# Wuziyi616/LEOD

Hardware: AMD Instinct MI355X
Metric: event-frames/sec/GPU (RVT-S train, Gen1 T=21) at 1/2/4/8 GPUs; mAP@0.5 parity (higher is better)
Workload: dtype fp16

## Files before the change

leod_amd/csrc/k_linear_wgrad.hip:

```cpp
#include "linear_common.hpp"
#include "wgrad_bf16.hpp"
#include "wgrad_dma.hpp"

LEOD_API long leod_workspace_bytes() { return (long)kWgwScratchBytes; }
LEOD_API int leod_set_workspace(void* ws, long bytes, hipStream_t stream) {
    if (ws && (bytes <= 0 || (reinterpret_cast<uintptr_t>(ws) & 15))) return LEOD_ERR_ARG;
    wgrad_wide_register_scratch(stream, ws, (size_t)(bytes > 0 ? bytes : 0));
    return LEOD_OK;
}

__global__ void leod_family_marker_kernel(int begin) { (void)begin; }
struct FamilyMarker {
    hipStream_t s; bool on;
    explicit FamilyMarker(hipStream_t st) : s(st) {
        static const bool env = getenv("LEOD_FAMILY_MARKERS") && atoi(getenv("LEOD_FAMILY_MARKERS"));
        on = env;
        if (on) hipLaunchKernelGGL(leod_family_marker_kernel, dim3(1), dim3(1), 0, s, 1);
    }
    ~FamilyMarker() { if (on) hipLaunchKernelGGL(leod_family_marker_kernel, dim3(1), dim3(1), 0, s, 0); }
};

static int route_linear_wgrad(const float* dy, long lddy, int dyfmt, const XRows& xl, float* dW, float* dbias, int M, int N, int K,
                              hipStream_t stream) {
    const int xm = xl.x_mode();
    if (xm == XM_BF16 || xm == XM_F16) {
        if (xl.stats || xl.x2) return LEOD_ERR_ARG;
        if (!use_wgrad_wide(xl, lddy, M, N, K, dyfmt) && !wgrad_dma_ok(xl, lddy, M, N, K, dyfmt)) return LEOD_ERR_UNSUPPORTED;
    }
    if (wgrad_dma_ok(xl, lddy, M, N, K, dyfmt)) {
        const int rc = launch_wgrad_dma(dy, lddy, xl, dW, (long)K, dbias, M, N, K, stream, dyfmt);
        if (rc != LEOD_ERR_UNSUPPORTED) return rc;
// ... 63 lines not shown
```

leod_amd/csrc/wgrad_bf16.hpp:

```cpp
#pragma once

typedef unsigned u4_ __attribute__((ext_vector_type(4)));

__device__ __forceinline__ f2_ gelu_erf2(f2_ x) {
    const f2_ z = __builtin_elementwise_abs(x) * 0.70710678118654752440f;
    const f2_ d = z * 0.3275911f + 1.0f;
    const f2_ t = {fast_rcp(d.x), fast_rcp(d.y)};
    const f2_ poly = t * (0.254829592f + t * (-0.284496736f + t * (1.421413741f + t * (-1.453152027f + t * 1.061405429f))));
    const f2_ a = (z * z) * -1.4426950408889634f;
    const f2_ e = {__builtin_amdgcn_exp2f(a.x), __builtin_amdgcn_exp2f(a.y)};
    const f2_ ht = (0.5f * poly) * e;
    const f2_ cdf = {x.x >= 0.f ? 1.0f - ht.x : ht.x, x.y >= 0.f ? 1.0f - ht.y : ht.y};
    return x * cdf;
}
__device__ __forceinline__ unsigned pack_bf16x2(f2_ v) { return __builtin_bit_cast(unsigned, __builtin_convertvector(v, bf2_)); }

constexpr int wgw_row_groups(int slots_per_row) {
    int g = 1;
    while (2 * g * slots_per_row <= 256) g *= 2;
    return g;
}
template <int RG, int T, int BST>
__device__ __forceinline__ constexpr int wgw_slot_off(int e) {
    return RG >= 16 ? e * (RG / 16) * T * BST : (e % (16 / (RG < 16 ? RG : 16))) * RG * 16 + (e / (16 / (RG < 16 ? RG : 16))) * T * BST;
}

template <int TN, int TK, int RC, int MS = 1>
constexpr int wgw_lds_bytes() {
    return 2 * ((RC / 16) * (TN + TK) * 272) * 2 > (MS - 1) * 12 * 1024 ? 2 * ((RC / 16) * (TN + TK) * 272) * 2 : (MS - 1) * 12 * 1024;
}

template <int TN, int TK, int NWN, int NWK, int RC, int DYF, int XM, int OCC>
__global__ __launch_bounds__(256, OCC) void wgrad_wide_bf16_kernel(const void* __restrict__ dyv, long lddy, XRows xl, float* dW, long ldw,
                                                                    float* dbias, f4* __restrict__ part, int M, int N, int K, int dbg) {
    constexpr int WA = TN / NWN, WB = TK / NWK, MS = 4 / (NWN * NWK), KS = RC / 32;
    constexpr bool K16 = KS % MS != 0;
    constexpr int NSL = WA * WB + WA;
    static_assert((WA == 3 || WA == 6) && (WB == 3 || WB == 6) && WA * WB <= 18 && NWN * NWK * MS == 4 && (RC / 16) % MS == 0 &&
                  (MS == 1 || (WA == 3 && WB == 3)), "4 waves of 3 x 3, 6 x 3 or 3 x 6 tiles");
    constexpr int BST = 16 * 16 + 16;
    constexpr int DCW = DYF ? 8 : 4, XCW = XM >= XM_GELU16 ? 8 : 4;
    constexpr int DSPR = 16 * TN / DCW, XSPR = 16 * TK / XCW;
    constexpr int DRG = wgw_row_groups(DSPR) < RC ? wgw_row_groups(DSPR) : RC, XRG = wgw_row_groups(XSPR) < RC ? wgw_row_groups(XSPR) : RC;
    constexpr bool XG = XM == XM_GELU16;
    static_assert(!XG || (RC * XSPR) % 256 == 0, "whole slots per thread");
    constexpr int RN = RC / DRG, RK = XG ? RC * XSPR / 256 : RC / XRG;
    constexpr int SDY = (RC / 16) * TN * BST, SX = (RC / 16) * TK * BST;
    static_assert(DSPR * DRG == 192 && (XG || XSPR * XRG == 192), "three waves stage an operand");
    static_assert(2 * (SDY + SX) * 2 <= wgw_lds_bytes<TN, TK, RC, MS>(), "LDS size");
    extern __shared__ __attribute__((aligned(16))) unsigned short wg_smem[];
    const int tid = threadIdx.x, lane = tid & 63, wave = __builtin_amdgcn_readfirstlane(tid >> 6);
    const int i = lane & 15, q = lane >> 4;
    const int wn = wave % NWN, wk = (wave / NWN) % NWK, ws = wave / (NWN * NWK);
    const int n0 = blockIdx.y * TN * 16, k0 = blockIdx.z * TK * 16;
    const bool dact = wave < 3, xact = XG || wave >= 1;
    const int xt = tid - 64;
    const int dcs = tid % DSPR, drg = tid / DSPR, xcs = (xact ? xt : 0) % XSPR, xrg = (xact ? xt : 0) / XSPR;
// ... 186 lines not shown
    }
    __syncthreads();
    int buf = 0;
    for (; m0 < M; m0 += mstride) {
        const long mn = m0 + mstride;
        const bool more = mn < M;
        if (more) { if (mn + RC <= M) fetch(mn, FULL); else fetch(mn, TAILC); }
        if (!(dbg & 2)) mfma_chunk(buf);
        if (more) stash(mn, buf ^ 1);
        __syncthreads();
        buf ^= 1;
    }
    if constexpr (MS > 1) {
        f4* sred = reinterpret_cast<f4*>(wg_smem);
        if (ws > 0) {
#pragma unroll
            for (int a = 0; a < WA; ++a) {
#pragma unroll
                for (int b = 0; b < WB; ++b) sred[((ws - 1) * NSL + a * WB + b) * 64 + lane] = acc[a][b];
                sred[((ws - 1) * NSL + WA * WB + a) * 64 + lane] = bacc[a];
            }
        }
        __syncthreads();
        if (ws > 0) return;
#pragma unroll
        for (int o = 0; o < MS - 1; ++o)
#pragma unroll
            for (int a = 0; a < WA; ++a) {
#pragma unroll
                for (int b = 0; b < WB; ++b) acc[a][b] += sred[(o * NSL + a * WB + b) * 64 + lane];
                bacc[a] += sred[(o * NSL + WA * WB + a) * 64 + lane];
            }
    }
    if (dbg & 1) return;
    if constexpr (XM == XM_LN) {
#pragma unroll
        for (int b = 0; b < WB; ++b) {
            const int k = k0 + 16 * (wk * WB + b) + i;
            const float g = k < K ? xl.ln_w[k] : 0.f, sh = k < K ? xl.ln_b[k] : 0.f;
#pragma unroll
            for (int a = 0; a < WA; ++a)
#pragma unroll
                for (int r = 0; r < 4; ++r) acc[a][b][r] = fmaf(g, acc[a][b][r], sh * bacc[a][r]);
        }
    }
    const bool bias_out = dbias != nullptr && blockIdx.z == 0;
    if (part != nullptr) {
        constexpr int NW = NWN * NWK;
        const long tile = (long)blockIdx.y * gridDim.z + blockIdx.z, ntiles = (long)gridDim.y * gridDim.z;
        f4* dst = part + (((long)blockIdx.x * ntiles + tile) * NW + (wk * NWN + wn)) * (NSL * 64) + lane;
#pragma unroll
        for (int a = 0; a < WA; ++a) {
#pragma unroll
            for (int b = 0; b < WB; ++b) dst[(a * WB + b) * 64] = acc[a][b];
            if (bias_out && a % NWK == wk) dst[(WA * WB + a) * 64] = bacc[a];
        }
        return;
    }
#pragma unroll
    for (int b = 0; b < WB; ++b) {
        const int k = k0 + 16 * (wk * WB + b) + i;
#pragma unroll
        for (int a = 0; a < WA; ++a)
#pragma unroll
            for (int r = 0; r < 4; ++r) {
                const int n = n0 + 16 * (wn * WA + a) + 4 * q + r;
                if (n < N && k < K) atomicAdd(dW + (long)n * ldw + k, acc[a][b][r]);
            }
    }
    if (bias_out && i == 0) {
#pragma unroll
        for (int a = 0; a < WA; ++a)
            if (a % NWK == wk) {
#pragma unroll
                for (int r = 0; r < 4; ++r) {
                    const int n = n0 + 16 * (wn * WA + a) + 4 * q + r;
                    if (n < N) atomicAdd(dbias + n, bacc[a][r]);
                }
            }
    }
}

template <int TN, int TK, int NWN, int NWK>
__global__ __launch_bounds__(256) void wgrad_wide_reduce_kernel(const f4* __restrict__ part, int gx, int ny, int nz, int per, float* dW, long ldw,
                                                                float* dbias, int N, int K) {
    constexpr int NW = NWN * NWK, WA = TN / NWN, WB = TK / NWK, NT9 = WA * WB, NSL = NT9 + WA;
    const long O = (long)ny * nz * NW * NSL * 64;
    const long o = (long)blockIdx.x * 256 + threadIdx.x;
    if (o >= O) return;
    const int lane = (int)(o & 63), t = (int)((o >> 6) % NSL), w = (int)((o / (64 * NSL)) % NW), tile = (int)(o / (64 * NSL * NW));
    const int ty = tile / nz, tz = tile - ty * nz, wn = w % NWN, wk = w / NWN, i = lane & 15, q = lane >> 4;
    if (t >= NT9 && !(dbias != nullptr && tz == 0 && (t - NT9) % NWK == wk && i == 0)) return;
    const int g0 = blockIdx.y * per, g1 = min(gx, g0 + per);
    f4 s0 = zero4(), s1 = zero4(), s2 = zero4(), s3 = zero4();
    const f4* p = part + (long)g0 * O + o;
    int g = g0;
    f4 s4 = zero4(), s5 = zero4(), s6 = zero4(), s7 = zero4();
    for (; g + 8 <= g1; g += 8, p += 8 * O) {
        s0 += p[0]; s1 += p[O]; s2 += p[2 * O]; s3 += p[3 * O]; s4 += p[4 * O]; s5 += p[5 * O]; s6 += p[6 * O]; s7 += p[7 * O];
    }
    for (; g + 4 <= g1; g += 4, p += 4 * O) { s0 += p[0]; s1 += p[O]; s2 += p[2 * O]; s3 += p[3 * O]; }
    for (; g < g1; ++g, p += O) s0 += p[0];
    const f4 v = ((s0 + s1) + (s2 + s3)) + ((s4 + s5) + (s6 + s7));
    const bool single = gridDim.y == 1;
    if (t < NT9) {
        const int a = t / WB, b = t - a * WB;
        const int k = tz * TK * 16 + 16 * (wk * WB + b) + i;
#pragma unroll
        for (int r = 0; r < 4; ++r) {
            const int n = ty * TN * 16 + 16 * (wn * WA + a) + 4 * q + r;
            if (n < N && k < K) {
                float* d = dW + (long)n * ldw + k;
                if (single) *d += v[r]; else atomicAdd(d, v[r]);
            }
        }
    } else {
#pragma unroll
        for (int r = 0; r < 4; ++r) {
            const int n = ty * TN * 16 + 16 * (wn * WA + (t - NT9)) + 4 * q + r;
            if (n < N) { if (single) dbias[n] += v[r]; else atomicAdd(dbias + n, v[r]); }
        }
    }
}

#include <mutex>
#include <unordered_map>
struct WgwScratch { void* p = nullptr; size_t bytes = 0; };
static inline std::unordered_map<hipStream_t, WgwScratch>& wgw_scratch_map() { static std::unordered_map<hipStream_t, WgwScratch> m; return m; }
static inline std::mutex& wgw_scratch_mutex() { static std::mutex m; return m; }
constexpr size_t kWgwScratchBytes = (size_t)768 << 20;
static inline void wgrad_wide_register_scratch(hipStream_t s, void* p, size_t bytes) {
    std::lock_guard<std::mutex> lock(wgw_scratch_mutex());
    WgwScratch& e = wgw_scratch_map()[s];
    e.p = p; e.bytes = p ? bytes : 0;
}
static inline f4* wgrad_wide_scratch(hipStream_t s, size_t bytes) {
    std::lock_guard<std::mutex> lock(wgw_scratch_mutex());
    WgwScratch& e = wgw_scratch_map()[s];
    if (e.bytes >= bytes) return reinterpret_cast<f4*>(e.p);
    hipStreamCaptureStatus cs = hipStreamCaptureStatusNone;
    if (hipStreamIsCapturing(s, &cs) != hipSuccess || cs != hipStreamCaptureStatusNone) { (void)hipGetLastError(); return nullptr; }
    void* nb = nullptr;
    const size_t want = bytes < kWgwScratchBytes ? kWgwScratchBytes : bytes;
    if (hipMalloc(&nb, want) != hipSuccess) { (void)hipGetLastError(); return nullptr; }
    e.p = nb; e.bytes = want;
    return reinterpret_cast<f4*>(nb);
}

template <int TN, int TK, int NWN, int NWK, int RC, int DYF, int XM, int OCC>
static inline int launch_wgrad_wide_cfg(const void* dy, long lddy, const XRows& xl, float* dW, long ldw, float* dbias,
                                        int M, int N, int K, hipStream_t s) {
    constexpr int dbg = 0;
    constexpr int LDS = wgw_lds_bytes<TN, TK, RC, 4 / (NWN * NWK)>();
    const int tiles = cdiv(N, TN * 16) * cdiv(K, TK * 16), chunks = cdiv(M, RC);
    const int wgs = M <= 60000 ? 384 : OCC * 256;
    int gx = max(1, min(chunks / 2, wgs / tiles));
    if (gx >= 16) gx &= ~7;
    dim3 grid(gx, cdiv(N, TN * 16), cdiv(K, TK * 16));
    auto kern = wgrad_wide_bf16_kernel<TN, TK, NWN, NWK, RC, DYF, XM, OCC>;
    static bool attr_set = false;
    if (!attr_set) { hipFuncSetAttribute(reinterpret_cast<const void*>(kern), hipFuncAttributeMaxDynamicSharedMemorySize, LDS); attr_set = true; }
    constexpr int NW = NWN * NWK, NSL = (TN / NWN) * (TK / NWK) + TN / NWN;
    const long O = (long)tiles * NW * NSL * 64;
    f4* part = gx > 1 ? wgrad_wide_scratch(s, (size_t)gx * O * sizeof(f4)) : nullptr;
    hipLaunchKernelGGL(kern, grid, dim3(256), LDS, s, dy, lddy, xl, dW, ldw, dbias, part, M, N, K, dbg);
    if (part != nullptr && !(dbg & 1)) {
        const int ob = (int)cdiv(O, 256);
        int groups = max(1, min(gx, 512 / ob));
        const int per = cdiv(gx, groups);
        groups = cdiv(gx, per);
        hipLaunchKernelGGL((wgrad_wide_reduce_kernel<TN, TK, NWN, NWK>), dim3(ob, groups), dim3(256), 0, s, part, gx, (int)grid.y, (int)grid.z, per,
                           dW, ldw, dbias, N, K);
    }
    return leod_launch_status();
}

static inline int wgrad_wide_combo(const XRows& xl, int N, int K, int dyfmt) {
    const int xm = xl.x_mode();
    if (xm == XM_F16) {
        if (dyfmt) return 0;
        if (N <= 48 && K <= 48) return 14;
        if (K <= 48 || N <= 48) return 0;
        return (K % 192 == 0 && N >= 96) ? 16 : 15;
    }
    const bool f32_rows = !dyfmt && xm == XM_ROWS, f32_gelu = !dyfmt && xm == XM_GELU16, f32_bf16 = !dyfmt && xm == XM_BF16;
    const bool b16_rows = dyfmt && xm == XM_ROWS, b16_ln = dyfmt && xm == XM_LN;
    if (N <= 48 && K <= 48) return f32_rows ? 1 : f32_bf16 ? 8 : 0;
    if (K <= 48) return b16_ln ? 2 : 0;
    if (N <= 48) return f32_gelu ? 3 : 0;
    if (N % 192 == 0 && K >= 96 && (b16_ln || b16_rows)) return b16_ln ? 10 : 11;
    if (K % 192 == 0 && N >= 96 && (f32_gelu || f32_bf16)) return f32_gelu ? 12 : 13;
    return f32_rows ? 4 : b16_ln ? 5 : f32_gelu ? 6 : b16_rows ? 7 : f32_bf16 ? 9 : 0;
}
static inline bool use_wgrad_wide(const XRows& xl, long lddy, int M, int N, int K, int dyfmt) {
    if (leod_precision() != 1 || M < 8192) return false;
    const int xm = xl.x_mode();
// ... 31 lines not shown
```

leod_amd/csrc/wgrad_dma.hpp:

```cpp
#pragma once

struct Prep16 {
    const void* src; long ld;
    const float* src2; long ld2; int C1;
    const float* stats;
    unsigned short* dst;
    int C, mode;
};
enum Prep16Mode : int { P16_NONE = -1, P16_F32 = 0, P16_LN = 1 , P16_GELU16 = 2, P16_F16 = 3, P16_CONCAT = 4  };
static inline int prep16_mode(int xm, bool concat) {
    if (xm_is_mfma_operand(xm)) return P16_NONE;
    return xm == XM_LN ? P16_LN : xm == XM_GELU16 ? P16_GELU16 : xm == XM_F16 ? P16_F16 : concat ? P16_CONCAT : P16_F32;
}

struct Prep16Group { Prep16 a[4]; Prep16 b[4]; };
__global__ __launch_bounds__(256) void wgrad_prep16_kernel(Prep16Group grp, int M) {
    const Prep16& p = blockIdx.y ? grp.b[blockIdx.z] : grp.a[blockIdx.z];
    if (p.mode < 0) return;
    const int C8 = p.C >> 3;
    const long it = (long)blockIdx.x * 256 + threadIdx.x;
    if (it >= (long)M * C8) return;
    const long m = it / C8;
    const int c = (int)(it - m * C8) << 3;
    f4 lo, hi;
// ... 6 lines not shown
    } else {
        const float* s = (p.mode == 4 && c >= p.C1) ? p.src2 + m * p.ld2 + (c - p.C1) : reinterpret_cast<const float*>(p.src) + m * p.ld + c;
        lo = ld4(s); hi = ld4(s + 4);
        if (p.mode == 1) {
            const f2_ st = *reinterpret_cast<const f2_*>(p.stats + 2 * m);
            lo = (lo - st.x) * st.y; hi = (hi - st.x) * st.y;
        }
    }
    const u4_ o = {pack_bf16x2(f2_{lo.x, lo.y}), pack_bf16x2(f2_{lo.z, lo.w}), pack_bf16x2(f2_{hi.x, hi.y}), pack_bf16x2(f2_{hi.z, hi.w})};
    *reinterpret_cast<u4_*>(p.dst + m * p.C + c) = o;
}

__device__ __forceinline__ void wgd_dma16(const void* gsrc, unsigned lds_dst) {
    unsigned keep;
    asm volatile("s_mov_b32 %0, m0\n\ts_mov_b32 m0, %2\n\ts_nop 0\n\tglobal_load_lds_dwordx4 %1, off\n\ts_mov_b32 m0, %0"
                 : "=&s"(keep) : "v"(gsrc), "s"(lds_dst) : "memory");
}
template <int N> __device__ __forceinline__ void wgd_wait_vm() { asm volatile("s_waitcnt vmcnt(%0)" :: "n"(N) : "memory"); }

template <int T, int RC, int NS> constexpr int wgd_lds_bytes() { return NS * 2 * (RC / 16) * T * 256 * 2; }
template <int T, int RC, int NS> constexpr int wgd_occupancy() { return wgd_lds_bytes<T, RC, NS>() <= 52 * 1024 ? 3 : wgd_lds_bytes<T, RC, NS>() <= 80 * 1024 ? 2 : 1; }

struct WgdProb {
    const unsigned short* A; long lda; const unsigned short* B; long ldb; const float* ln_w; const float* ln_b; float* dbias_flag; f4* part;
    int cpw, gx, ny, nz, N, K, blk0;
};
struct WgdGroup { WgdProb p[4]; int n; };
template <int T, int RC, int NS, bool LN>
__global__ __launch_bounds__(256, ((wgd_occupancy<T, RC, NS>()) >= 2 ? 2 : 1)) void wgrad_dma_kernel(WgdGroup grp, int chunks, int dbg) {
    int pk = 0;
    for (int k = 1; k < grp.n; ++k) if ((int)blockIdx.x >= grp.p[k].blk0) pk = k;
    const WgdProb& pr = grp.p[pk];
    const unsigned short* __restrict__ A = pr.A; const unsigned short* __restrict__ B = pr.B; const long lda = pr.lda, ldb = pr.ldb;
    const float* __restrict__ ln_w = pr.ln_w; const float* __restrict__ ln_b = pr.ln_b; float* dbias_flag = pr.dbias_flag; f4* __restrict__ part = pr.part;
    const int cpw = pr.cpw, gx = pr.gx, ny = pr.ny, nz = pr.nz, K = pr.K;
    const int bid = (int)blockIdx.x - pr.blk0;
    const bool ln = LN && ln_w != nullptr;
    constexpr int WA = T / 2, WB = T / 2, NWN = 2, NWK = 2, RB = RC / 16, KS = RC / 32;
    constexpr int BLK = 256;
    constexpr int SA = RB * T * BLK, SLOT = 2 * SA;
    constexpr int NI = SLOT * 2 / 1024, IPW = NI / 4;
    static_assert(NI % 4 == 0 && RC % 32 == 0, "whole instructions per wave");
    constexpr int NSL = WA * WB + WA;
    extern __shared__ __attribute__((aligned(1024))) unsigned short wd_smem[];
    const int tid = threadIdx.x, lane = tid & 63, wave = __builtin_amdgcn_readfirstlane(tid >> 6);
    const int i = lane & 15, q = lane >> 4;
    const int wn = wave % NWN, wk = wave / NWN;
    const int ntl = ny * nz;
    int tl, bx;
    if ((gx & 7) == 0) { const int xcd = bid & 7, sj = bid >> 3; tl = sj % ntl; bx = (sj / ntl) * 8 + xcd; }
    else { bx = bid % gx; tl = bid / gx; }
    const int by = tl / nz, bz = tl - by * nz;
    const int n0 = by * T * 16, k0 = bz * T * 16;
    const int c0 = bx * cpw, c1 = min(chunks, c0 + cpw);
    const int nch = c1 - c0;
    static_assert(IPW % 2 == 0, "the first half of a wave's instructions fills the dY part, the second half the X part");
    const char* src[IPW];
    const long stepA = (long)RC * lda * 2, stepB = (long)RC * ldb * 2;
#pragma unroll
    for (int j = 0; j < IPW; ++j) {
        const int t = wave + 4 * j;
        const int blk = 2 * t + (lane >> 5), r = (lane & 31) >> 1, half = lane & 1;
        const bool isb = j >= IPW / 2;
        const int b = isb ? blk - RB * T : blk;
        const int rb = b / T, cb = b - rb * T;
        const long ld = isb ? ldb : lda;
        const int col = (isb ? k0 : n0) + cb * 16 + half * 8;
        src[j] = reinterpret_cast<const char*>(isb ? B : A) + (((long)c0 * RC + rb * 16 + r) * ld + col) * 2;
    }
    const unsigned lds0 = __builtin_amdgcn_readfirstlane((unsigned)(size_t)wd_smem);
    auto issue = [&](int slot) {
#pragma unroll
        for (int j = 0; j < IPW; ++j) {
            wgd_dma16(src[j], __builtin_amdgcn_readfirstlane(lds0 + (unsigned)(slot * SLOT * 2 + (wave + 4 * j) * 1024)));
            src[j] += j >= IPW / 2 ? stepB : stepA;
        }
    };
    const bool bias_out = dbias_flag != nullptr && bz == 0;
    const bool bias_any = ln || bias_out;
    f4 acc[WA][WB], bacc[WA];
#pragma unroll
    for (int a = 0; a < WA; ++a) {
        bacc[a] = zero4();
#pragma unroll
        for (int b = 0; b < WB; ++b) acc[a][b] = zero4();
    }
    const s8v ones = {0x3F80, 0x3F80, 0x3F80, 0x3F80, 0x3F80, 0x3F80, 0x3F80, 0x3F80};
    typedef __attribute__((address_space(3))) s4 lds_s4;
    const int loff = (4 * q + (i >> 2)) * 16 + 4 * (i & 3);
    auto mfma_chunk = [&](int slot) {
        const unsigned short* pdy = wd_smem + slot * SLOT + (wn * WA) * BLK + loff;
        const unsigned short* px = wd_smem + slot * SLOT + SA + (wk * WB) * BLK + loff;
#pragma unroll
        for (int ks = 0; ks < KS; ++ks) {
            const int st = 2 * ks;
            s8v pa[WA], pb[WB];
#pragma unroll
            for (int a = 0; a < WA; ++a) {
                const s4 lo = __builtin_amdgcn_ds_read_tr16_b64_v4i16((lds_s4*)(pdy + (st * T + a) * BLK));
                const s4 hi = __builtin_amdgcn_ds_read_tr16_b64_v4i16((lds_s4*)(pdy + ((st + 1) * T + a) * BLK));
                pa[a] = __builtin_shufflevector(lo, hi, 0, 1, 2, 3, 4, 5, 6, 7);
// ... 25 lines not shown
        if (c + NS - 1 < nch && !(dbg & 2)) issue((c + NS - 1) % NS);
        if (!(dbg & 1)) mfma_chunk(c % NS);
    }
    if (ln) {
#pragma unroll
        for (int b = 0; b < WB; ++b) {
            const int k = k0 + 16 * (wk * WB + b) + i;
            const float g = k < K ? ln_w[k] : 0.f, sh = k < K ? ln_b[k] : 0.f;
#pragma unroll
            for (int a = 0; a < WA; ++a)
#pragma unroll
                for (int r = 0; r < 4; ++r) acc[a][b][r] = fmaf(g, acc[a][b][r], sh * bacc[a][r]);
        }
    }
    constexpr int NW = NWN * NWK;
    const long tile = (long)by * nz + bz, ntiles = ntl;
    f4* dst = part + (((long)bx * ntiles + tile) * NW + (wk * NWN + wn)) * (NSL * 64) + lane;
#pragma unroll
    for (int a = 0; a < WA; ++a) {
#pragma unroll
        for (int b = 0; b < WB; ++b) dst[(a * WB + b) * 64] = acc[a][b];
        if (bias_out && a % NWK == wk) dst[(WA * WB + a) * 64] = bacc[a];
    }
}

constexpr int kWgdRC = 64;
constexpr size_t kWgdOperandBytes = (size_t)600 << 20;

static inline int wgd_tile(int N, int K) {
    if (N % 96 == 0 && K % 96 == 0) return 6;
    if (N % 128 == 0 && K % 128 == 0) return 8;
    if (N % 64 == 0 && K % 64 == 0) return 4;
    return 0;
}
static inline bool wgrad_dma_ok(const XRows& xl, long lddy, int M, int N, int K, int dyfmt) {
    if (leod_precision() != 1 || M < 8192 || (M % kWgdRC) || N < 64 || K < 64) return false;
    const int T = wgd_tile(N, K);
    if (!T) return false;
    const int xm = xl.x_mode();
    if ((lddy & 7) || (xl.ld & 7)) return false;
    if (xl.x2 && (xm != XM_ROWS || (xl.K1 & 7) || (xl.ld2 & 7))) return false;
    const size_t need = (size_t)M * ((dyfmt ? 0 : N) + (xm_is_mfma_operand(xm) ? 0 : K)) * 2;
    if (need > kWgdOperandBytes) return false;
    if (M > (T == 6 ? 60000 : 400000)) return false;
    if (!dyfmt && xm != XM_BF16 && xm != XM_GELU16 && (long)N * K < 200000) return false;
    return true;
}

struct WgrProb { const f4* part; float* dW; float* dbias; long ldw; int gx, ny, nz, per, N, K, ob, groups; };
struct WgrGroup { WgrProb p[4]; };
template <int T>
__global__ __launch_bounds__(256) void wgrad_dma_reduce_kernel(WgrGroup grp) {
    const WgrProb& pr = grp.p[blockIdx.z];
    if ((int)blockIdx.x >= pr.ob || (int)blockIdx.y >= pr.groups) return;
    constexpr int NWN = 2, NWK = 2, NW = 4, WA = T / 2, WB = T / 2, NT9 = WA * WB, NSL = NT9 + WA;
    const int gx = pr.gx, nz = pr.nz, per = pr.per, N = pr.N, K = pr.K;
    float* dW = pr.dW; float* dbias = pr.dbias; const long ldw = pr.ldw;
    const long O = (long)pr.ny * nz * NW * NSL * 64;
    const long o = (long)blockIdx.x * 256 + threadIdx.x;
    if (o >= O) return;
    const int lane = (int)(o & 63), t = (int)((o >> 6) % NSL), w = (int)((o / (64 * NSL)) % NW), tile = (int)(o / (64 * NSL * NW));
    const int ty = tile / nz, tz = tile - ty * nz, wn = w % NWN, wk = w / NWN, i = lane & 15, q = lane >> 4;
    if (t >= NT9 && !(dbias != nullptr && tz == 0 && (t - NT9) % NWK == wk && i == 0)) return;
    const int g0 = blockIdx.y * per, g1 = min(gx, g0 + per);
    f4 s0 = zero4(), s1 = zero4(), s2 = zero4(), s3 = zero4(), s4 = zero4(), s5 = zero4(), s6 = zero4(), s7 = zero4();
    const f4* p = pr.part + (long)g0 * O + o;
    int g = g0;
    for (; g + 8 <= g1; g += 8, p += 8 * O) {
        s0 += p[0]; s1 += p[O]; s2 += p[2 * O]; s3 += p[3 * O]; s4 += p[4 * O]; s5 += p[5 * O]; s6 += p[6 * O]; s7 += p[7 * O];
    }
    for (; g + 4 <= g1; g += 4, p += 4 * O) { s0 += p[0]; s1 += p[O]; s2 += p[2 * O]; s3 += p[3 * O]; }
    for (; g < g1; ++g, p += O) s0 += p[0];
    const f4 v = ((s0 + s1) + (s2 + s3)) + ((s4 + s5) + (s6 + s7));
    const bool single = pr.groups == 1;
    if (t < NT9) {
        const int a = t / WB, b = t - a * WB;
        const int k = tz * T * 16 + 16 * (wk * WB + b) + i;
#pragma unroll
        for (int r = 0; r < 4; ++r) {
            const int n = ty * T * 16 + 16 * (wn * WA + a) + 4 * q + r;
            if (n < N && k < K) {
                float* d = dW + (long)n * ldw + k;
                if (single) *d += v[r]; else atomicAdd(d, v[r]);
            }
        }
    } else {
#pragma unroll
        for (int r = 0; r < 4; ++r) {
            const int n = ty * T * 16 + 16 * (wn * WA + (t - NT9)) + 4 * q + r;
            if (n < N) { if (single) dbias[n] += v[r]; else atomicAdd(dbias + n, v[r]); }
        }
    }
}

struct WgdHostProb { const void* dy; long lddy; XRows xl; float* dW; long ldw; float* dbias; int N, K, dyfmt; };

template <int T, int RC, int NS>
static inline int launch_wgrad_dma_group_t(int n, const WgdHostProb* hp, int M, hipStream_t s) {
    constexpr int TW = T * 16;
    constexpr int LDS = wgd_lds_bytes<T, RC, NS>();
    constexpr int dbg = 0;
    constexpr int NW = 4, NSL = (T / 2) * (T / 2) + T / 2;
    const int chunks = M / RC;
    const int target = 256 * wgd_occupancy<T, RC, NS>();
    int total_tiles = 0;
    for (int k = 0; k < n; ++k) total_tiles += (hp[k].N / TW) * (hp[k].K / TW);
    WgdGroup g{};
    WgrGroup rg{};
    Prep16Group pg{};
    size_t off = 0, offs_part[4], offs_a[4], offs_b[4];
    int blk = 0, obmax = 0, grmax = 0, c8max = 0;
    bool any_ln = false, any_prep = false;
    for (int k = 0; k < n; ++k) {
        const WgdHostProb& h = hp[k];
        const int xm = h.xl.x_mode();
        const int tiles = (h.N / TW) * (h.K / TW);
        int gx = max(1, min(chunks / NS, target / total_tiles));
        if (gx >= 8) gx &= ~7;
        const int cpw = cdiv(chunks, gx);
        if (gx < 8) gx = cdiv(chunks, cpw);
        const long O = (long)tiles * NW * NSL * 64;
        offs_part[k] = off; off += ((size_t)gx * O * sizeof(f4) + 1023) & ~(size_t)1023;
        offs_a[k] = off; off += h.dyfmt ? 0 : (((size_t)M * h.N * 2 + 1023) & ~(size_t)1023);
        offs_b[k] = off; off += xm_is_mfma_operand(xm) ? 0 : (((size_t)M * h.K * 2 + 1023) & ~(size_t)1023);
        g.p[k].cpw = cpw; g.p[k].gx = gx; g.p[k].ny = h.N / TW; g.p[k].nz = h.K / TW; g.p[k].N = h.N; g.p[k].K = h.K; g.p[k].blk0 = blk;
        blk += gx * tiles;
        const int ob = (int)cdiv(O, 256);
        int groups = max(1, min(gx, 512 / ob));
        const int per = cdiv(gx, groups);
        groups = cdiv(gx, per);
        rg.p[k] = WgrProb{nullptr, h.dW, h.dbias, h.ldw, gx, h.N / TW, h.K / TW, per, h.N, h.K, ob, groups};
        obmax = max(obmax, ob); grmax = max(grmax, groups);
        any_ln = any_ln || xm == XM_LN;
    }
    g.n = n;
    char* ws = reinterpret_cast<char*>(wgrad_wide_scratch(s, off + 4096));
    if (!ws) return LEOD_ERR_UNSUPPORTED;
    for (int k = 0; k < n; ++k) {
        const WgdHostProb& h = hp[k];
        const int xm = h.xl.x_mode();
        f4* part = reinterpret_cast<f4*>(ws + offs_part[k]);
        unsigned short* a16 = reinterpret_cast<unsigned short*>(ws + offs_a[k]);
        unsigned short* b16 = reinterpret_cast<unsigned short*>(ws + offs_b[k]);
        Prep16 pa{}, pb{};
        pa.mode = pb.mode = P16_NONE;
        if (!h.dyfmt) pa = Prep16{h.dy, h.lddy, nullptr, 0, 0, nullptr, a16, h.N, P16_F32};
        if (!xm_is_mfma_operand(xm)) pb = Prep16{h.xl.x, h.xl.ld, h.xl.x2, h.xl.ld2, h.xl.x2 ? h.xl.K1 : h.K, h.xl.stats, b16, h.K,
                                                 prep16_mode(xm, h.xl.x2 != nullptr)};
        pg.a[k] = pa; pg.b[k] = pb;
        if (pa.mode >= 0) { any_prep = true; c8max = max(c8max, h.N / 8); }
        if (pb.mode >= 0) { any_prep = true; c8max = max(c8max, h.K / 8); }
        g.p[k].A = h.dyfmt ? reinterpret_cast<const unsigned short*>(h.dy) : a16;
        g.p[k].lda = h.dyfmt ? h.lddy : h.N;
        g.p[k].B = xm_is_mfma_operand(xm) ? reinterpret_cast<const unsigned short*>(h.xl.x) : b16;
        g.p[k].ldb = xm_is_mfma_operand(xm) ? h.xl.ld : h.K;
        g.p[k].ln_w = xm == XM_LN ? h.xl.ln_w : nullptr; g.p[k].ln_b = xm == XM_LN ? h.xl.ln_b : nullptr;
        g.p[k].dbias_flag = h.dbias; g.p[k].part = part;
        rg.p[k].part = part;
    }
    for (int k = n; k < 4; ++k) { pg.a[k].mode = pg.b[k].mode = P16_NONE; }
    if (any_prep) hipLaunchKernelGGL(wgrad_prep16_kernel, dim3(cdiv((long)M * c8max, 256), 2, n), dim3(256), 0, s, pg, M);
    if (any_ln) {
        auto kern = wgrad_dma_kernel<T, RC, NS, true>;
        static bool attr_set = false;
        if (!attr_set) { hipFuncSetAttribute(reinterpret_cast<const void*>(kern), hipFuncAttributeMaxDynamicSharedMemorySize, LDS); attr_set = true; }
        hipLaunchKernelGGL(kern, dim3(blk), dim3(256), LDS, s, g, chunks, dbg);
    } else {
        auto kern = wgrad_dma_kernel<T, RC, NS, false>;
        static bool attr_set = false;
        if (!attr_set) { hipFuncSetAttribute(reinterpret_cast<const void*>(kern), hipFuncAttributeMaxDynamicSharedMemorySize, LDS); attr_set = true; }
        hipLaunchKernelGGL(kern, dim3(blk), dim3(256), LDS, s, g, chunks, dbg);
    }
    hipLaunchKernelGGL(wgrad_dma_reduce_kernel<T>, dim3(obmax, grmax, n), dim3(256), 0, s, rg);
    return leod_launch_status();
}
template <int T, int RC, int NS>
static inline int launch_wgrad_dma_t(const void* dy, long lddy, const XRows& xl, float* dW, long ldw, float* dbias,
                                     int M, int N, int K, hipStream_t s, int dyfmt) {
    const WgdHostProb h{dy, lddy, xl, dW, ldw, dbias, N, K, dyfmt};
    return launch_wgrad_dma_group_t<T, RC, NS>(1, &h, M, s);
}
static inline int launch_wgrad_dma(const void* dy, long lddy, const XRows& xl, float* dW, long ldw, float* dbias,
                                   int M, int N, int K, hipStream_t s, int dyfmt) {
    switch (wgd_tile(N, K)) {
        case 6: return launch_wgrad_dma_t<6, 64, 3>(dy, lddy, xl, dW, ldw, dbias, M, N, K, s, dyfmt);
        case 8: return launch_wgrad_dma_t<8, 64, 2>(dy, lddy, xl, dW, ldw, dbias, M, N, K, s, dyfmt);
        default: return launch_wgrad_dma_t<4, 64, 3>(dy, lddy, xl, dW, ldw, dbias, M, N, K, s, dyfmt);
    }
}
```

leod_amd/ops.py:

```python
from typing import Optional, Sequence, Tuple

import ctypes

import torch

from ._lib import lib, check, LeodHipError, DevPtr

F32 = torch.float32


_LIB = None


def _l():
    global _LIB
    if _LIB is None:
        _LIB = lib()
    return _LIB


try:
    _raw_stream = torch._C._cuda_getCurrentRawStream
except AttributeError:
    _raw_stream = None
# ... 1279 lines not shown
    def dump(self, path: str):
        check(_l().leod_plan_dump(self.handle, path.encode()), 'plan_dump')

    def close(self):
        if getattr(self, 'handle', 0):
            _l().leod_plan_destroy(self.handle)
            self.handle = 0
        self.graph = None

    def __del__(self):
        try:
            self.close()
        except Exception:
            pass

_PROBE = None


class KernelProbe:

    def __init__(self, targets=('linear_wgrad', 'linear_gemm'), kernel_names=None, families=True):
        global _PROBE, _LIB
        self.targets = tuple(targets)
        self.kernel_names = kernel_names or {'linear_wgrad': 'wgrad_wide_bf16_kernel + wgrad_wide_reduce_kernel (bf16 mode) / wgradw_kernel<.., XRows> (f32 mode)',
                                             'linear_gemm': 'rowstream* / gemm_lds_kernel / gemm_wide_bf16_kernel (Linear forward + dgrad)'}
        self.step = 0
        self.events = {t: [] for t in self.targets}
        self.fam_events = {}
        self.calls = []
        self.real_lib = _l()
        if families:
            _LIB = _ProbedLib(self.real_lib, self)
        _PROBE = self

    def mark_step(self):
        self.step += 1

    @property
    def steps(self):
        return max(self.step, 1)

    def begin(self, target, nbytes, flops=0.0, rows=None, nbytes16=None):
        e0, e1 = torch.cuda.Event(enable_timing=True), torch.cuda.Event(enable_timing=True)
        e0.record()
        self.events[target].append((self.step, e0, e1, nbytes, flops, nbytes if nbytes16 is None else nbytes16, rows))
        return e1

# ... 106 lines not shown
```

Measured before the change: 11290.

## Fuse split-K wgrad reduction into GEMM kernels via last-arriving-block counters

Removes the separate reduce kernel launches for the wide bf16 and DMA weight-gradient paths. Each block writes its partials, then increments a per-tile counter kept in the workspace, and the last block to arrive for a tile group sums the partials and writes dW/dbias. This saves a kernel launch and the tail-to-head gap between the two kernels. In exchange it adds atomic counters, fences and a serialized tail reduction done by one block per group, and it reserves 64KB of counters that are zeroed once at registration and reset by the last block.

```diff
diff --git a/leod_amd/csrc/k_linear_wgrad.hip b/leod_amd/csrc/k_linear_wgrad.hip
--- a/leod_amd/csrc/k_linear_wgrad.hip
+++ b/leod_amd/csrc/k_linear_wgrad.hip
@@ -5,8 +5,7 @@
 LEOD_API long leod_workspace_bytes() { return (long)kWgwScratchBytes; }
 LEOD_API int leod_set_workspace(void* ws, long bytes, hipStream_t stream) {
     if (ws && (bytes <= 0 || (reinterpret_cast<uintptr_t>(ws) & 15))) return LEOD_ERR_ARG;
-    wgrad_wide_register_scratch(stream, ws, (size_t)(bytes > 0 ? bytes : 0));
-    return LEOD_OK;
+    return wgrad_wide_register_scratch(stream, ws, (size_t)(bytes > 0 ? bytes : 0));
 }
 
 __global__ void leod_family_marker_kernel(int begin) { (void)begin; }
diff --git a/leod_amd/csrc/wgrad_bf16.hpp b/leod_amd/csrc/wgrad_bf16.hpp
--- a/leod_amd/csrc/wgrad_bf16.hpp
+++ b/leod_amd/csrc/wgrad_bf16.hpp
@@ -30,9 +30,74 @@
     return 2 * ((RC / 16) * (TN + TK) * 272) * 2 > (MS - 1) * 12 * 1024 ? 2 * ((RC / 16) * (TN + TK) * 272) * 2 : (MS - 1) * 12 * 1024;
 }
 
+constexpr size_t kWgCounterBytes = (size_t)64 << 10;
+constexpr int kWgCounters = (int)(kWgCounterBytes / sizeof(unsigned));
+__device__ __forceinline__ bool wgrad_arrive_last(unsigned* cnt, int expect, unsigned* flag) {
+    asm volatile("s_waitcnt vmcnt(0)" ::: "memory");
+    __syncthreads();
+    if (threadIdx.x == 0) {
+        __builtin_amdgcn_fence(__ATOMIC_RELEASE, "agent");
+        asm volatile("s_waitcnt vmcnt(0)" ::: "memory");
+        const unsigned old = __hip_atomic_fetch_add(cnt, 1u, __ATOMIC_RELAXED, __HIP_MEMORY_SCOPE_AGENT);
+        const bool last = old == (unsigned)(expect - 1);
+        if (last) {
+            __hip_atomic_store(cnt, 0u, __ATOMIC_RELAXED, __HIP_MEMORY_SCOPE_AGENT);
+            __builtin_amdgcn_fence(__ATOMIC_ACQUIRE, "agent");
+            asm volatile("s_waitcnt vmcnt(0)" ::: "memory");
+        }
+        *flag = last ? 1u : 0u;
+    }
+    __syncthreads();
+    return *flag != 0u;
+}
+template <int WA, int WB, int NWN, int NWK>
+__device__ __forceinline__ void wgrad_reduce_tile(const f4* part, long ntiles, long tile, int g0, int g1, bool single, float* dW, long ldw,
+                                                  float* dbias, int n0, int k0, int N, int K) {
+    constexpr int NW = NWN * NWK, NT9 = WA * WB, NSL = NT9 + WA, TS = NW * NSL * 64;
+    const long O = ntiles * TS;
+    const int lane = threadIdx.x & 63, i = lane & 15, q = lane >> 4;
+    for (int sl = threadIdx.x >> 6; sl < NW * NSL; sl += 4) {
+        const int w = sl / NSL, t = sl - w * NSL, wn = w % NWN, wk = w / NWN;
+        if (t >= NT9 && !(dbias != nullptr && (t - NT9) % NWK == wk && i == 0)) continue;
+        const f4* p = part + (long)g0 * O + tile * TS + sl * 64 + lane;
+        f4 s0 = zero4(), s1 = zero4(), s2 = zero4(), s3 = zero4(), s4 = zero4(), s5 = zero4(), s6 = zero4(), s7 = zero4();
+        int g = g0;
+        for (; g + 8 <= g1; g += 8, p += 8 * O) {
+            s0 += p[0]; s1 += p[O]; s2 += p[2 * O]; s3 += p[3 * O]; s4 += p[4 * O]; s5 += p[5 * O]; s6 += p[6 * O]; s7 += p[7 * O];
+        }
+        for (; g + 4 <= g1; g += 4, p += 4 * O) { s0 += p[0]; s1 += p[O]; s2 += p[2 * O]; s3 += p[3 * O]; }
+        for (; g < g1; ++g, p += O) s0 += p[0];
+        const f4 v = ((s0 + s1) + (s2 + s3)) + ((s4 + s5) + (s6 + s7));
+        if (t < NT9) {
+            const int a = t / WB, b = t - a * WB;
+            const int k = k0 + 16 * (wk * WB + b) + i;
+#pragma unroll
+            for (int r = 0; r < 4; ++r) {
+                const int n = n0 + 16 * (wn * WA + a) + 4 * q + r;
+                if (n < N && k < K) {
+                    float* d = dW + (long)n * ldw + k;
+                    if (single) *d += v[r]; else atomicAdd(d, v[r]);
+                }
+            }
+        } else {
+#pragma unroll
+            for (int r = 0; r < 4; ++r) {
+                const int n = n0 + 16 * (wn * WA + (t - NT9)) + 4 * q + r;
+                if (n < N) { if (single) dbias[n] += v[r]; else atomicAdd(dbias + n, v[r]); }
+            }
+        }
+    }
+}
+static inline int wgrad_reduce_per(int gx, long O, int tiles) {
+    const int ob = (int)cdiv(O, 256);
+    int groups = max(1, min(gx, 512 / ob));
+    groups = max(1, min(groups, kWgCounters / tiles));
+    return cdiv(gx, groups);
+}
+
 template <int TN, int TK, int NWN, int NWK, int RC, int DYF, int XM, int OCC>
 __global__ __launch_bounds__(256, OCC) void wgrad_wide_bf16_kernel(const void* __restrict__ dyv, long lddy, XRows xl, float* dW, long ldw,
-                                                                    float* dbias, f4* __restrict__ part, int M, int N, int K, int dbg) {
+                                                                    float* dbias, f4* part, unsigned* cnt, int per, int M, int N, int K, int dbg) {
     constexpr int WA = TN / NWN, WB = TK / NWK, MS = 4 / (NWN * NWK), KS = RC / 32;
     constexpr bool K16 = KS % MS != 0;
     constexpr int NSL = WA * WB + WA;
@@ -265,15 +330,17 @@
             }
         }
         __syncthreads();
-        if (ws > 0) return;
-#pragma unroll
-        for (int o = 0; o < MS - 1; ++o)
-#pragma unroll
-            for (int a = 0; a < WA; ++a) {
-#pragma unroll
-                for (int b = 0; b < WB; ++b) acc[a][b] += sred[(o * NSL + a * WB + b) * 64 + lane];
-                bacc[a] += sred[(o * NSL + WA * WB + a) * 64 + lane];
-            }
+        if (ws > 0 && part == nullptr) return;
+        if (ws == 0) {
+#pragma unroll
+            for (int o = 0; o < MS - 1; ++o)
+#pragma unroll
+                for (int a = 0; a < WA; ++a) {
+#pragma unroll
+                    for (int b = 0; b < WB; ++b) acc[a][b] += sred[(o * NSL + a * WB + b) * 64 + lane];
+                    bacc[a] += sred[(o * NSL + WA * WB + a) * 64 + lane];
+                }
+        }
     }
     if (dbg & 1) return;
     if constexpr (XM == XM_LN) {
@@ -292,12 +359,18 @@
         constexpr int NW = NWN * NWK;
         const long tile = (long)blockIdx.y * gridDim.z + blockIdx.z, ntiles = (long)gridDim.y * gridDim.z;
         f4* dst = part + (((long)blockIdx.x * ntiles + tile) * NW + (wk * NWN + wn)) * (NSL * 64) + lane;
-#pragma unroll
-        for (int a = 0; a < WA; ++a) {
-#pragma unroll
-            for (int b = 0; b < WB; ++b) dst[(a * WB + b) * 64] = acc[a][b];
-            if (bias_out && a % NWK == wk) dst[(WA * WB + a) * 64] = bacc[a];
-        }
+        if (ws == 0) {
+#pragma unroll
+            for (int a = 0; a < WA; ++a) {
+#pragma unroll
+                for (int b = 0; b < WB; ++b) dst[(a * WB + b) * 64] = acc[a][b];
+                if (bias_out && a % NWK == wk) dst[(WA * WB + a) * 64] = bacc[a];
+            }
+        }
+        const int gx = (int)gridDim.x, groups = (gx + per - 1) / per, grp = (int)blockIdx.x / per;
+        const int g0 = grp * per, g1 = min(gx, g0 + per);
+        if (!wgrad_arrive_last(cnt + tile * groups + grp, g1 - g0, reinterpret_cast<unsigned*>(wg_smem))) return;
+        wgrad_reduce_tile<WA, WB, NWN, NWK>(part, ntiles, tile, g0, g1, groups == 1, dW, ldw, bias_out ? dbias : nullptr, n0, k0, N, K);
         return;
     }
 #pragma unroll
@@ -321,48 +394,6 @@
                     if (n < N) atomicAdd(dbias + n, bacc[a][r]);
                 }
             }
-    }
-}
-
-template <int TN, int TK, int NWN, int NWK>
-__global__ __launch_bounds__(256) void wgrad_wide_reduce_kernel(const f4* __restrict__ part, int gx, int ny, int nz, int per, float* dW, long ldw,
-                                                                float* dbias, int N, int K) {
-    constexpr int NW = NWN * NWK, WA = TN / NWN, WB = TK / NWK, NT9 = WA * WB, NSL = NT9 + WA;
-    const long O = (long)ny * nz * NW * NSL * 64;
-    const long o = (long)blockIdx.x * 256 + threadIdx.x;
-    if (o >= O) return;
-    const int lane = (int)(o & 63), t = (int)((o >> 6) % NSL), w = (int)((o / (64 * NSL)) % NW), tile = (int)(o / (64 * NSL * NW));
-    const int ty = tile / nz, tz = tile - ty * nz, wn = w % NWN, wk = w / NWN, i = lane & 15, q = lane >> 4;
-    if (t >= NT9 && !(dbias != nullptr && tz == 0 && (t - NT9) % NWK == wk && i == 0)) return;
-    const int g0 = blockIdx.y * per, g1 = min(gx, g0 + per);
-    f4 s0 = zero4(), s1 = zero4(), s2 = zero4(), s3 = zero4();
-    const f4* p = part + (long)g0 * O + o;
-    int g = g0;
-    f4 s4 = zero4(), s5 = zero4(), s6 = zero4(), s7 = zero4();
-    for (; g + 8 <= g1; g += 8, p += 8 * O) {
-        s0 += p[0]; s1 += p[O]; s2 += p[2 * O]; s3 += p[3 * O]; s4 += p[4 * O]; s5 += p[5 * O]; s6 += p[6 * O]; s7 += p[7 * O];
-    }
-    for (; g + 4 <= g1; g += 4, p += 4 * O) { s0 += p[0]; s1 += p[O]; s2 += p[2 * O]; s3 += p[3 * O]; }
-    for (; g < g1; ++g, p += O) s0 += p[0];
-    const f4 v = ((s0 + s1) + (s2 + s3)) + ((s4 + s5) + (s6 + s7));
-    const bool single = gridDim.y == 1;
-    if (t < NT9) {
-        const int a = t / WB, b = t - a * WB;
-        const int k = tz * TK * 16 + 16 * (wk * WB + b) + i;
-#pragma unroll
-        for (int r = 0; r < 4; ++r) {
-            const int n = ty * TN * 16 + 16 * (wn * WA + a) + 4 * q + r;
-            if (n < N && k < K) {
-                float* d = dW + (long)n * ldw + k;
-                if (single) *d += v[r]; else atomicAdd(d, v[r]);
-            }
-        }
-    } else {
-#pragma unroll
-        for (int r = 0; r < 4; ++r) {
-            const int n = ty * TN * 16 + 16 * (wn * WA + (t - NT9)) + 4 * q + r;
-            if (n < N) { if (single) dbias[n] += v[r]; else atomicAdd(dbias + n, v[r]); }
-        }
     }
 }
 
@@ -372,22 +403,31 @@
 static inline std::unordered_map<hipStream_t, WgwScratch>& wgw_scratch_map() { static std::unordered_map<hipStream_t, WgwScratch> m; return m; }
 static inline std::mutex& wgw_scratch_mutex() { static std::mutex m; return m; }
 constexpr size_t kWgwScratchBytes = (size_t)768 << 20;
-static inline void wgrad_wide_register_scratch(hipStream_t s, void* p, size_t bytes) {
+static inline int wgrad_wide_register_scratch(hipStream_t s, void* p, size_t bytes) {
     std::lock_guard<std::mutex> lock(wgw_scratch_mutex());
     WgwScratch& e = wgw_scratch_map()[s];
-    e.p = p; e.bytes = p ? bytes : 0;
-}
-static inline f4* wgrad_wide_scratch(hipStream_t s, size_t bytes) {
+    e.p = nullptr; e.bytes = 0;
+    if (!p) return LEOD_OK;
+    if (bytes <= kWgCounterBytes) return LEOD_ERR_ARG;
+    if (hipMemsetAsync(p, 0, kWgCounterBytes, s) != hipSuccess) { (void)hipGetLastError(); return LEOD_ERR_LAUNCH; }
+    e.p = p; e.bytes = bytes;
+    return LEOD_OK;
+}
+struct WgwSpace { unsigned* cnt; f4* scratch; };
+static inline WgwSpace wgrad_wide_scratch(hipStream_t s, size_t bytes) {
     std::lock_guard<std::mutex> lock(wgw_scratch_mutex());
     WgwScratch& e = wgw_scratch_map()[s];
-    if (e.bytes >= bytes) return reinterpret_cast<f4*>(e.p);
-    hipStreamCaptureStatus cs = hipStreamCaptureStatusNone;
-    if (hipStreamIsCapturing(s, &cs) != hipSuccess || cs != hipStreamCaptureStatusNone) { (void)hipGetLastError(); return nullptr; }
-    void* nb = nullptr;
-    const size_t want = bytes < kWgwScratchBytes ? kWgwScratchBytes : bytes;
-    if (hipMalloc(&nb, want) != hipSuccess) { (void)hipGetLastError(); return nullptr; }
-    e.p = nb; e.bytes = want;
-    return reinterpret_cast<f4*>(nb);
+    bytes += kWgCounterBytes;
+    if (e.bytes < bytes) {
+        hipStreamCaptureStatus cs = hipStreamCaptureStatusNone;
+        if (hipStreamIsCapturing(s, &cs) != hipSuccess || cs != hipStreamCaptureStatusNone) { (void)hipGetLastError(); return WgwSpace{nullptr, nullptr}; }
+        void* nb = nullptr;
+        const size_t want = bytes < kWgwScratchBytes ? kWgwScratchBytes : bytes;
+        if (hipMalloc(&nb, want) != hipSuccess) { (void)hipGetLastError(); return WgwSpace{nullptr, nullptr}; }
+        if (hipMemsetAsync(nb, 0, kWgCounterBytes, s) != hipSuccess) { (void)hipGetLastError(); (void)hipFree(nb); return WgwSpace{nullptr, nullptr}; }
+        e.p = nb; e.bytes = want;
+    }
+    return WgwSpace{reinterpret_cast<unsigned*>(e.p), reinterpret_cast<f4*>(reinterpret_cast<char*>(e.p) + kWgCounterBytes)};
 }
 
 template <int TN, int TK, int NWN, int NWK, int RC, int DYF, int XM, int OCC>
@@ -405,16 +445,9 @@
     if (!attr_set) { hipFuncSetAttribute(reinterpret_cast<const void*>(kern), hipFuncAttributeMaxDynamicSharedMemorySize, LDS); attr_set = true; }
     constexpr int NW = NWN * NWK, NSL = (TN / NWN) * (TK / NWK) + TN / NWN;
     const long O = (long)tiles * NW * NSL * 64;
-    f4* part = gx > 1 ? wgrad_wide_scratch(s, (size_t)gx * O * sizeof(f4)) : nullptr;
-    hipLaunchKernelGGL(kern, grid, dim3(256), LDS, s, dy, lddy, xl, dW, ldw, dbias, part, M, N, K, dbg);
-    if (part != nullptr && !(dbg & 1)) {
-        const int ob = (int)cdiv(O, 256);
-        int groups = max(1, min(gx, 512 / ob));
-        const int per = cdiv(gx, groups);
-        groups = cdiv(gx, per);
-        hipLaunchKernelGGL((wgrad_wide_reduce_kernel<TN, TK, NWN, NWK>), dim3(ob, groups), dim3(256), 0, s, part, gx, (int)grid.y, (int)grid.z, per,
-                           dW, ldw, dbias, N, K);
-    }
+    const WgwSpace sp = gx > 1 ? wgrad_wide_scratch(s, (size_t)gx * O * sizeof(f4)) : WgwSpace{nullptr, nullptr};
+    const int per = sp.scratch ? wgrad_reduce_per(gx, O, tiles) : 1;
+    hipLaunchKernelGGL(kern, grid, dim3(256), LDS, s, dy, lddy, xl, dW, ldw, dbias, sp.scratch, sp.cnt, per, M, N, K, dbg);
     return leod_launch_status();
 }
 
diff --git a/leod_amd/csrc/wgrad_dma.hpp b/leod_amd/csrc/wgrad_dma.hpp
--- a/leod_amd/csrc/wgrad_dma.hpp
+++ b/leod_amd/csrc/wgrad_dma.hpp
@@ -52,8 +52,9 @@
 template <int T, int RC, int NS> constexpr int wgd_occupancy() { return wgd_lds_bytes<T, RC, NS>() <= 52 * 1024 ? 3 : wgd_lds_bytes<T, RC, NS>() <= 80 * 1024 ? 2 : 1; }
 
 struct WgdProb {
-    const unsigned short* A; long lda; const unsigned short* B; long ldb; const float* ln_w; const float* ln_b; float* dbias_flag; f4* part;
-    int cpw, gx, ny, nz, N, K, blk0;
+    const unsigned short* A; long lda; const unsigned short* B; long ldb; const float* ln_w; const float* ln_b; float* dbias; f4* part;
+    float* dW; long ldw; unsigned* cnt;
+    int cpw, gx, ny, nz, N, K, blk0, per;
 };
 struct WgdGroup { WgdProb p[4]; int n; };
 template <int T, int RC, int NS, bool LN>
@@ -62,8 +63,8 @@
     for (int k = 1; k < grp.n; ++k) if ((int)blockIdx.x >= grp.p[k].blk0) pk = k;
     const WgdProb& pr = grp.p[pk];
     const unsigned short* __restrict__ A = pr.A; const unsigned short* __restrict__ B = pr.B; const long lda = pr.lda, ldb = pr.ldb;
-    const float* __restrict__ ln_w = pr.ln_w; const float* __restrict__ ln_b = pr.ln_b; float* dbias_flag = pr.dbias_flag; f4* __restrict__ part = pr.part;
-    const int cpw = pr.cpw, gx = pr.gx, ny = pr.ny, nz = pr.nz, K = pr.K;
+    const float* __restrict__ ln_w = pr.ln_w; const float* __restrict__ ln_b = pr.ln_b; float* dbias = pr.dbias; f4* part = pr.part;
+    const int cpw = pr.cpw, gx = pr.gx, ny = pr.ny, nz = pr.nz, N = pr.N, K = pr.K, per = pr.per;
     const int bid = (int)blockIdx.x - pr.blk0;
     const bool ln = LN && ln_w != nullptr;
     constexpr int WA = T / 2, WB = T / 2, NWN = 2, NWK = 2, RB = RC / 16, KS = RC / 32;
@@ -106,7 +107,7 @@
             src[j] += j >= IPW / 2 ? stepB : stepA;
         }
     };
-    const bool bias_out = dbias_flag != nullptr && bz == 0;
+    const bool bias_out = dbias != nullptr && bz == 0;
     const bool bias_any = ln || bias_out;
     f4 acc[WA][WB], bacc[WA];
 #pragma unroll
@@ -178,6 +179,10 @@
         for (int b = 0; b < WB; ++b) dst[(a * WB + b) * 64] = acc[a][b];
         if (bias_out && a % NWK == wk) dst[(WA * WB + a) * 64] = bacc[a];
     }
+    const int groups = (gx + per - 1) / per, rgrp = bx / per;
+    const int g0 = rgrp * per, g1 = min(gx, g0 + per);
+    if (!wgrad_arrive_last(pr.cnt + tile * groups + rgrp, g1 - g0, reinterpret_cast<unsigned*>(wd_smem))) return;
+    wgrad_reduce_tile<WA, WB, NWN, NWK>(part, ntiles, tile, g0, g1, groups == 1, pr.dW, pr.ldw, bias_out ? dbias : nullptr, n0, k0, N, K);
 }
 
 constexpr int kWgdRC = 64;
@@ -203,52 +208,6 @@
     return true;
 }
 
-struct WgrProb { const f4* part; float* dW; float* dbias; long ldw; int gx, ny, nz, per, N, K, ob, groups; };
-struct WgrGroup { WgrProb p[4]; };
-template <int T>
-__global__ __launch_bounds__(256) void wgrad_dma_reduce_kernel(WgrGroup grp) {
-    const WgrProb& pr = grp.p[blockIdx.z];
-    if ((int)blockIdx.x >= pr.ob || (int)blockIdx.y >= pr.groups) return;
-    constexpr int NWN = 2, NWK = 2, NW = 4, WA = T / 2, WB = T / 2, NT9 = WA * WB, NSL = NT9 + WA;
-    const int gx = pr.gx, nz = pr.nz, per = pr.per, N = pr.N, K = pr.K;
-    float* dW = pr.dW; float* dbias = pr.dbias; const long ldw = pr.ldw;
-    const long O = (long)pr.ny * nz * NW * NSL * 64;
-    const long o = (long)blockIdx.x * 256 + threadIdx.x;
-    if (o >= O) return;
-    const int lane = (int)(o & 63), t = (int)((o >> 6) % NSL), w = (int)((o / (64 * NSL)) % NW), tile = (int)(o / (64 * NSL * NW));
-    const int ty = tile / nz, tz = tile - ty * nz, wn = w % NWN, wk = w / NWN, i = lane & 15, q = lane >> 4;
-    if (t >= NT9 && !(dbias != nullptr && tz == 0 && (t - NT9) % NWK == wk && i == 0)) return;
-    const int g0 = blockIdx.y * per, g1 = min(gx, g0 + per);
-    f4 s0 = zero4(), s1 = zero4(), s2 = zero4(), s3 = zero4(), s4 = zero4(), s5 = zero4(), s6 = zero4(), s7 = zero4();
-    const f4* p = pr.part + (long)g0 * O + o;
-    int g = g0;
-    for (; g + 8 <= g1; g += 8, p += 8 * O) {
-        s0 += p[0]; s1 += p[O]; s2 += p[2 * O]; s3 += p[3 * O]; s4 += p[4 * O]; s5 += p[5 * O]; s6 += p[6 * O]; s7 += p[7 * O];
-    }
-    for (; g + 4 <= g1; g += 4, p += 4 * O) { s0 += p[0]; s1 += p[O]; s2 += p[2 * O]; s3 += p[3 * O]; }
-    for (; g < g1; ++g, p += O) s0 += p[0];
-    const f4 v = ((s0 + s1) + (s2 + s3)) + ((s4 + s5) + (s6 + s7));
-    const bool single = pr.groups == 1;
-    if (t < NT9) {
-        const int a = t / WB, b = t - a * WB;
-        const int k = tz * T * 16 + 16 * (wk * WB + b) + i;
-#pragma unroll
-        for (int r = 0; r < 4; ++r) {
-            const int n = ty * T * 16 + 16 * (wn * WA + a) + 4 * q + r;
-            if (n < N && k < K) {
-                float* d = dW + (long)n * ldw + k;
-                if (single) *d += v[r]; else atomicAdd(d, v[r]);
-            }
-        }
-    } else {
-#pragma unroll
-        for (int r = 0; r < 4; ++r) {
-            const int n = ty * T * 16 + 16 * (wn * WA + (t - NT9)) + 4 * q + r;
-            if (n < N) { if (single) dbias[n] += v[r]; else atomicAdd(dbias + n, v[r]); }
-        }
-    }
-}
-
 struct WgdHostProb { const void* dy; long lddy; XRows xl; float* dW; long ldw; float* dbias; int N, K, dyfmt; };
 
 template <int T, int RC, int NS>
@@ -262,10 +221,10 @@
     int total_tiles = 0;
     for (int k = 0; k < n; ++k) total_tiles += (hp[k].N / TW) * (hp[k].K / TW);
     WgdGroup g{};
-    WgrGroup rg{};
     Prep16Group pg{};
     size_t off = 0, offs_part[4], offs_a[4], offs_b[4];
-    int blk = 0, obmax = 0, grmax = 0, c8max = 0;
+    int offs_cnt[4];
+    int blk = 0, ncnt = 0, c8max = 0;
     bool any_ln = false, any_prep = false;
     for (int k = 0; k < n; ++k) {
         const WgdHostProb& h = hp[k];
@@ -281,17 +240,15 @@
         offs_b[k] = off; off += xm_is_mfma_operand(xm) ? 0 : (((size_t)M * h.K * 2 + 1023) & ~(size_t)1023);
         g.p[k].cpw = cpw; g.p[k].gx = gx; g.p[k].ny = h.N / TW; g.p[k].nz = h.K / TW; g.p[k].N = h.N; g.p[k].K = h.K; g.p[k].blk0 = blk;
         blk += gx * tiles;
-        const int ob = (int)cdiv(O, 256);
-        int groups = max(1, min(gx, 512 / ob));
-        const int per = cdiv(gx, groups);
-        groups = cdiv(gx, per);
-        rg.p[k] = WgrProb{nullptr, h.dW, h.dbias, h.ldw, gx, h.N / TW, h.K / TW, per, h.N, h.K, ob, groups};
-        obmax = max(obmax, ob); grmax = max(grmax, groups);
+        const int per = wgrad_reduce_per(gx, O, 4 * tiles);
+        g.p[k].per = per; g.p[k].dW = h.dW; g.p[k].ldw = h.ldw;
+        offs_cnt[k] = ncnt; ncnt += tiles * cdiv(gx, per);
         any_ln = any_ln || xm == XM_LN;
     }
     g.n = n;
-    char* ws = reinterpret_cast<char*>(wgrad_wide_scratch(s, off + 4096));
-    if (!ws) return LEOD_ERR_UNSUPPORTED;
+    const WgwSpace sp = wgrad_wide_scratch(s, off + 4096);
+    char* ws = reinterpret_cast<char*>(sp.scratch);
+    if (!ws || ncnt > kWgCounters) return LEOD_ERR_UNSUPPORTED;
     for (int k = 0; k < n; ++k) {
         const WgdHostProb& h = hp[k];
         const int xm = h.xl.x_mode();
@@ -311,8 +268,7 @@
         g.p[k].B = xm_is_mfma_operand(xm) ? reinterpret_cast<const unsigned short*>(h.xl.x) : b16;
         g.p[k].ldb = xm_is_mfma_operand(xm) ? h.xl.ld : h.K;
         g.p[k].ln_w = xm == XM_LN ? h.xl.ln_w : nullptr; g.p[k].ln_b = xm == XM_LN ? h.xl.ln_b : nullptr;
-        g.p[k].dbias_flag = h.dbias; g.p[k].part = part;
-        rg.p[k].part = part;
+        g.p[k].dbias = h.dbias; g.p[k].part = part; g.p[k].cnt = sp.cnt + offs_cnt[k];
     }
     for (int k = n; k < 4; ++k) { pg.a[k].mode = pg.b[k].mode = P16_NONE; }
     if (any_prep) hipLaunchKernelGGL(wgrad_prep16_kernel, dim3(cdiv((long)M * c8max, 256), 2, n), dim3(256), 0, s, pg, M);
@@ -327,7 +283,6 @@
         if (!attr_set) { hipFuncSetAttribute(reinterpret_cast<const void*>(kern), hipFuncAttributeMaxDynamicSharedMemorySize, LDS); attr_set = true; }
         hipLaunchKernelGGL(kern, dim3(blk), dim3(256), LDS, s, g, chunks, dbg);
     }
-    hipLaunchKernelGGL(wgrad_dma_reduce_kernel<T>, dim3(obmax, grmax, n), dim3(256), 0, s, rg);
     return leod_launch_status();
 }
 template <int T, int RC, int NS>
diff --git a/leod_amd/ops.py b/leod_amd/ops.py
--- a/leod_amd/ops.py
+++ b/leod_amd/ops.py
@@ -1325,7 +1325,7 @@
     def __init__(self, targets=('linear_wgrad', 'linear_gemm'), kernel_names=None, families=True):
         global _PROBE, _LIB
         self.targets = tuple(targets)
-        self.kernel_names = kernel_names or {'linear_wgrad': 'wgrad_wide_bf16_kernel + wgrad_wide_reduce_kernel (bf16 mode) / wgradw_kernel<.., XRows> (f32 mode)',
+        self.kernel_names = kernel_names or {'linear_wgrad': 'wgrad_wide_bf16_kernel / wgrad_dma_kernel (16-bit modes) / wgradw_kernel<.., XRows> (f32 mode)',
                                              'linear_gemm': 'rowstream* / gemm_lds_kernel / gemm_wide_bf16_kernel (Linear forward + dgrad)'}
         self.step = 0
         self.events = {t: [] for t in self.targets}
```

New measurement: 10740. 0.951x the previous value.
